# swift-nav/albatross

Hardware: AMD Instinct MI355X
Metric: GP fits/sec (Gram+Chol+solve) at N=16384 fp64 (higher is better)
Workload: dtype f64

## Files before the change

albatross_amd/csrc/api.hip:

```cpp
#include <algorithm>
#include <atomic>
#include <cmath>
#include <cstring>
#include <chrono>
#include <cstdio>
#include <new>
#include <thread>

#include "api_internal.h"
#include "batch_front.h"
#include <deque>
#include <mutex>
#include <tuple>
#include <unordered_map>
#include "trace.h"
#include "pub.h"

namespace agp {

void DeviceFeatures::release() {
  for (void *&p : owned) {
    if (p) (void)hipFree(p);
    p = nullptr;
  }
// ... 138 lines not shown
  return n;
}

static constexpr long long BACKSUB_COOP_MAX_N = 2047;
static agp_context::Tuning read_tuning() {
  agp_context::Tuning t;
  auto flag = [](const char *name, bool dflt) {
    const char *e = getenv(name);
    return e && e[0] ? e[0] == '1' : dflt;
  };
  auto number = [](const char *name, long long dflt) {
    const char *e = getenv(name);
    return e && e[0] ? atoll(e) : dflt;
  };
  t.panel_fused = flag("AGP_PANEL_FUSED", true);
  t.step_below = number("AGP_STEP_BELOW", 4608);
  t.gram_sop = flag("AGP_GRAM_SOP", true);
  t.backsub_coop = flag("AGP_BACKSUB_COOP", true);
  t.backsub_coop_max = number("AGP_BACKSUB_COOP_MAX", BACKSUB_COOP_MAX_N);
  t.mixed_bf16 = flag("AGP_MIXED_BF16", true);
  t.mixed_f16 = flag("AGP_MIXED_F16", true);
  set_f16x2_kernel((int)number("AGP_F16X2_LDS_PAD", 8192), (int)number("AGP_F16X2_TERMS", 4), (int)number("AGP_F16X2_CHUNK", 32));
  t.mixed_nbo = number("AGP_MIXED_NBO", 512);
  t.fp64_nbo = number("AGP_FP64_NBO", 0);
  if (t.fp64_nbo <= 512 || t.fp64_nbo % 128 != 0) t.fp64_nbo = 0;
  set_bf16x3_kernel((int)number("AGP_BF16X3_KERNEL", 2), (int)number("AGP_BF16X3_LDS_PAD", 8192));
  t.sparse_pivoted = flag("AGP_SPARSE_PIVOTED", false);
  t.predict_chunk = number("AGP_PREDICT_CHUNK", 0);
  t.shard_block = number("AGP_SHARD_BLOCK", 0);
  t.shard_force_comm = flag("AGP_SHARD_FORCE_COMM", false);
  t.shard_host_pacing = flag("AGP_SHARD_HOST_PACING", false);
  if (const char *e = getenv("AGP_SHARD_MASK_GFLOP")) t.shard_mask_gflop = atof(e);
  t.merge_above = number("AGP_MERGE_ABOVE", 8704);
  return t;
}

int agp_context_create(int device_id, agp_context **out) {
  if (!out) return AGP_ERR_INVALID_ARGUMENT;
  *out = nullptr;
  int n = 0;
  if (hipGetDeviceCount(&n) != hipSuccess || n <= 0) return AGP_ERR_NO_DEVICE;
  if (device_id < 0 || device_id >= n) return AGP_ERR_INVALID_ARGUMENT;
  agp_context_impl *ctx = new (std::nothrow) agp_context_impl();
  if (!ctx) return AGP_ERR_INVALID_ARGUMENT;
  ctx->device = device_id;
  ctx->tune = read_tuning();
  agp::g_gram_sop = ctx->tune.gram_sop;
  AGP_HIP_CHECK(ctx, hipSetDevice(device_id));
  {
    int lo = 0, hi = 0;
    AGP_HIP_CHECK(ctx, hipDeviceGetStreamPriorityRange(&lo, &hi));
    AGP_HIP_CHECK(ctx, hipStreamCreateWithPriority(&ctx->stream, hipStreamNonBlocking, hi));
    AGP_HIP_CHECK(ctx, hipStreamCreateWithPriority(&ctx->stream2, hipStreamNonBlocking, lo));
    AGP_HIP_CHECK(ctx, hipStreamCreateWithPriority(&ctx->stream3, hipStreamNonBlocking, lo));
    AGP_HIP_CHECK(ctx, hipEventCreateWithFlags(&ctx->ev_inv, hipEventDisableTiming));
    AGP_HIP_CHECK(ctx, hipEventCreateWithFlags(&ctx->ev_c, hipEventDisableTiming));
    int cus = 256;
    (void)hipDeviceGetAttribute(&cus, hipDeviceAttributeMultiprocessorCount, device_id);
    ctx->cus = cus;
    const int keep = cus / 8 * 7 / 8 * 8;
    if (keep > 0 && keep < cus) {
      uint32_t mask[16] = {0};
      for (int i = 0; i < keep && i < 512; ++i) mask[i / 32] |= 1u << (i % 32);
      if (hipExtStreamCreateWithCUMask(&ctx->stream_masked, (uint32_t)((cus + 31) / 32), mask) != hipSuccess) {
        (void)hipGetLastError();
        ctx->stream_masked = nullptr;
// ... 1693 lines not shown
```

albatross_amd/csrc/chol.hip:

```cpp
#include <cstdlib>
#include "common.h"
#include "mfma_f64.h"
#include "gemm_tiles.h"
#include "trsm_kernel.h"
#include "pub.h"
#include "factor_plan.h"

namespace agp {
void launch_set_identity_batched(hipStream_t s, double *B, long long ld, long long stride, long long m, long long count);

__device__ __forceinline__ double readlane_f64(double v, int lane) {
  const long long b = __double_as_longlong(v);
  const int lo = __builtin_amdgcn_readlane((int)(b & 0xffffffffll), lane);
  const int hi = __builtin_amdgcn_readlane((int)(b >> 32), lane);
  return __longlong_as_double(((long long)hi << 32) | (unsigned int)lo);
}

__device__ __forceinline__ double rsqrt_nr(double x) {
  double y = __builtin_amdgcn_rsq(x);
  const double h = 0.5 * x;
  y = y * (1.5 - h * y * y);
  y = y * (1.5 - h * y * y);
  return y;
}
// ... 795 lines not shown
    ctx->d_rowcnt = nullptr;
    ctx->dpub_cap = 0;
    const long long cap = (b1 + 31) / 32 * 32;
    if (hipMalloc(&ctx->d_dpub, sizeof(double) * (size_t)cap * (IMG_DOUBLES + 2)) == hipSuccess) {
      ctx->dpub_cap = cap;
      ctx->d_rowcnt = reinterpret_cast<unsigned long long *>(ctx->d_dpub + cap * (long long)IMG_DOUBLES);
    }
    else (void)hipGetLastError();
  }
  const long long cnt_img = (b1 - b0) * (long long)IMG_DOUBLES, cnt_z = k_end - k_begin;
  if (ctx->d_dpub && ctx->dpub_cap >= b1) {
    prep->fill(ctx->d_rowcnt + 2 * b0, 0ull, 2 * (b1 - b0));
    prep->sentinel(ctx->d_dpub + b0 * (long long)IMG_DOUBLES, cnt_img);
  }
  prep->sentinel(invd + b0 * (long long)IMG_DOUBLES, cnt_img);
  prep->sentinel(ctx->d_zpub + k_begin, cnt_z);
  if (want_step && k_begin == 0 && ctx->d_headcnt && ctx->tune.merge_above > 0 && k_end > ctx->tune.merge_above && !prep->full()) {
    prep->fill(ctx->d_headcnt, 0ull, agp_context::HEADCNT_WORDS);
    ctx->headcnt_ready = true;
  }
  ctx->zpub_ready_n = k_end;
  ctx->img_ready = invd;
  return true;
}

void panel_fused_prepare(agp_context *ctx, hipStream_t s, double *invd, long long k_begin, long long k_end, bool want_step) {
  PrepArgs prep;
  if (panel_fused_plan(ctx, invd, k_begin, k_end, want_step, &prep)) launch_prep(s, prep);
}

static FactorSwitches factor_switches(agp_context *ctx, const double *invd, long long upto, int variant) {
  FactorSwitches sw;
  sw.panel_fused = ctx->tune.panel_fused; sw.step_below = ctx->tune.step_below; sw.merge_above = ctx->tune.merge_above;
  sw.nbo_override = ctx->nbo_override;
  sw.nbo_wide = (variant == 4 || variant == 5) ? ctx->nbo_wide : ctx->tune.fp64_nbo;
  sw.variant = variant;
  sw.step_slots = sw.step_below > 0 ? step_slots(ctx) : 0;
  sw.cus = ctx->cus;
  sw.have_masked_stream = ctx->stream_masked != nullptr;
  sw.headcnt_ready = ctx->headcnt_ready;
  sw.fused_buffers_ready = ctx->d_zpub && ctx->zpub_ready_n >= upto && ctx->img_ready == invd;
  sw.step_buffers_ready = sw.panel_fused && sw.fused_buffers_ready && ctx->d_dpub && ctx->dpub_cap * NB >= upto && ctx->d_rowcnt;
  sw.inv_requested = ctx->bs_W && ctx->ev_inv && ctx->stream2;
  sw.bs_BW = ctx->bs_BW; sw.bs_done = ctx->bs_done;
  return sw;
}

static void panel_phase(agp_context *ctx, hipStream_t s, double *A, long long n, long long lda, double *invd,
                        double *y, long long K0, long long kend, FactorTimers *timers, const FactorSwitches &sw,
                        bool want_step = false, long long mark_after = -1, hipEvent_t mark_event = nullptr) {
  const PanelPlan pp = plan_panels(n, K0, kend, want_step, sw);
  const bool step_mode = pp.step_mode, inner_left = pp.inner_left, fused = pp.fused;
  for (long long k = K0; k < kend; k += NB) {
    const int nbk = (int)((n - k < NB) ? n - k : NB);
    if (mark_event && k == mark_after + NB) (void)hipEventRecord(mark_event, s);
    if (inner_left && k > K0) {
      const double *P = A + K0 * lda + k;
      timed_gemm(s, timers, A + k * lda + k, lda, P, P, n - k, nbk, k - K0, false);
    }
    const long long below = n - (k + nbk);
    if (fused) {
      PotrfArgs pa;
      pa.A = A; pa.lda = lda; pa.k0 = k; pa.nbk = nbk;
      pa.img = invd + (k / NB) * (long long)IMG_DOUBLES;
      pa.y = y ? y + k : nullptr;
      pa.flags = ctx->d_flags; pa.scalars = ctx->d_scalars;
      pa.zpub = y ? ctx->d_zpub + k : nullptr;
      pa.below = below > 0 ? below : 0;
      if (step_mode && k > K0) {
        pa.dpub = ctx->d_dpub + (k / NB) * (long long)IMG_DOUBLES;
        const StepLaunchShape sh = step_launch_shape(pa.below, (k - K0) / NB, sw.step_slots, sw.cus);
        pa.trail_first = sh.trail_first; pa.trail_tiles = sh.trail_tiles; pa.trail_workers = sh.trail_workers;
        pa.hold_index = sh.hold_index; pa.hold_count = sh.hold_count;
        pa.rowcnt_expect = sh.rowcnt_expect;
        if (pa.below > 0) pa.rowcnt = ctx->d_rowcnt + (k + NB) / 64;
        hipLaunchKernelGGL(panel_fused_kernel<true>, dim3(sh.grid), dim3(256), 0, s, pa);
        ++ctx->sched.panels_step;
      } else {
        hipLaunchKernelGGL(panel_fused_kernel<false>, dim3((unsigned)(1 + (pa.below + 63) / 64)), dim3(256), 0, s, pa);
        ++ctx->sched.panels_fused;
      }
      if (below <= 0) continue;
    } else {
      launch_potrf(s, A, lda, k, nbk, invd, y, ctx->d_flags, ctx->d_scalars);
      ++ctx->sched.panels_split;
      if (below <= 0) continue;
      TrsmArgs t;
      t.img = invd + (k / NB) * (long long)IMG_DOUBLES;
      t.nbk = nbk;
      t.Y = A + k * lda + (k + nbk);
      t.stride_m = lda; t.stride_n = 1;
// ... 362 lines not shown
```

albatross_amd/csrc/common.h:

```cpp
#pragma once
#include <hip/hip_runtime.h>
#include <cstdint>
#include <cstdio>
#include <string>
#include <type_traits>
#include <utility>
#include <vector>

#include "../../include/albatross_amd.h"
#include "cov_eval.h"

#define AGP_CHAIN_PRIO 3

namespace agp {

constexpr int NB = 128;
constexpr int NBO = 512;
constexpr int MB = 16;
constexpr int NMB = NB / MB;

template <class F>
inline void dispatch_dim(int dim, F &&f) {
  if (dim == 1) f(std::integral_constant<int, 1>{});
  else if (dim == 2) f(std::integral_constant<int, 2>{});
// ... 55 lines not shown
  size_t pool_aux_bytes = 0;
  int update_variant = -1;
  long long nbo_override = 0;
  long long nbo_wide = 0;
  double *pool_shard = nullptr;
  size_t pool_shard_bytes = 0;
  double *pool_sparse = nullptr;
  size_t pool_sparse_bytes = 0;
  double *pool_batch = nullptr;
  size_t pool_batch_bytes = 0;
  double *d_zpub = nullptr;
  long long zpub_cap = 0, zpub_ready_n = 0;
  double *d_dpub = nullptr;
  long long dpub_cap = 0;
  int cus = 256;
  long long step_slots = 0;
  struct Tuning {
    bool panel_fused = true;
    long long step_below = 4608;
    bool gram_sop = true;
    long long fp64_nbo = 0;
    long long mixed_nbo = 512;
    bool mixed_f16 = true;
    bool mixed_bf16 = true;
    long long backsub_coop_max = 2047;
    bool backsub_coop = true;
    bool sparse_pivoted = false;
    long long predict_chunk = 0;
    long long shard_block = 0;
    bool shard_force_comm = false;
    bool shard_host_pacing = false;
    double shard_mask_gflop = 40.;
    long long merge_above = 8704;
  } tune;
  unsigned long long *d_rowcnt = nullptr;
  void *h_stage = nullptr;
  size_t h_stage_bytes = 0;
  static constexpr long long HEADCNT_WORDS = 256;
  unsigned long long *d_headcnt = nullptr;
  bool headcnt_ready = false;
  struct ScheduleRecord {
    static constexpr unsigned MERGED = 1, STEP = 2, THROTTLED = 4, MASKED = 8, SINGLE = 16;
    enum Backsub { BS_NONE = 0, BS_COOP_DIRECT = 1, BS_COOP_FLAGS = 2, BS_WIDE = 3, BS_CHAIN = 4 };
    static constexpr unsigned INV_EARLY = 1, INV_LAST_STEP = 2, INV_TAIL = 4;
    long long n = 0;
    long long steps = 0, steps_dropped = 0;
    long long kend[HEADCNT_WORDS] = {};
    unsigned bits[HEADCNT_WORDS] = {};
    long long panels_step = 0, panels_fused = 0, panels_split = 0;
    int backsub = BS_NONE;
    long long bs_done = 0;
    unsigned inv_bits = 0;
    int handover_timeout = 0;
    long long demotions = 0;
    void reset_factor(long long n_) {
      n = n_;
      steps = steps_dropped = 0;
      panels_step = panels_fused = panels_split = 0;
      inv_bits = 0;
      handover_timeout = 0;
    }
    void add_step(long long end, unsigned b) {
      if (steps < HEADCNT_WORDS) { kend[steps] = end; bits[steps] = b; ++steps; }
      else ++steps_dropped;
    }
  } sched;
  double *bs_W = nullptr;
  long long bs_BW = 0, bs_done = 0;
  hipEvent_t ev_inv = nullptr;
  const double *img_ready = nullptr;
  bool prep_external = false;
  hipStream_t stream_comm = nullptr;
  unsigned long long *shard_flags = nullptr;
  unsigned long long shard_seq[16] = {};
  unsigned long long shard_probe_seq = 0;
  int shard_host_pacing = -1;
  bool shard_probe_ok = false;
};

struct agp_fit_slab {
  double *base = nullptr;
  size_t bytes = 0;
  int refs = 0;
};

struct agp_fit {
  agp_context *ctx = nullptr;
  agp_fit_slab *slab = nullptr;
  size_t A_bytes = 0;
  int device = 0;
  int64_t n = 0;
// ... 89 lines not shown
void right_solve_lt_batched(hipStream_t s, const double *A, long long stride_A, long long n, long long lda,
                            const double *invd, long long stride_invd, double *X, long long stride_X, long long nrows,
                            long long ldx, long long count);
void launch_gemm_nt_sub_batched(hipStream_t s, double *C, long long ldc, long long batch_C, const double *A,
                                long long lda, bool a_kmajor, long long batch_A, const double *B, long long ldb,
                                bool b_kmajor, long long batch_B, long long M, long long N, long long K, bool tri,
                                long long count);
void right_solve_lt(hipStream_t s, const double *A, long long n, long long lda, const double *invd, double *X,
                    long long nrows, long long ldx);
void forward_solve_mat_lookahead(agp_context *ctx, const double *A, long long n, long long lda, const double *invd,
                                 double *B, long long m, long long ldb, bool rhs_lower = false);
void backward_solve_mat(hipStream_t s, const double *A, long long n, long long lda, const double *invd,
                        double *B, long long m, long long ldb);
constexpr long long WIDE_BW = 512;
bool forward_solve_wide_ok(long long n, long long ncols);
void invert_wide_blocks(hipStream_t s, const double *A, long long n, long long lda, const double *invd, long long BW, double *W);
void forward_solve_wide(hipStream_t s, const double *A, long long n, long long lda, const double *Winv, const double *B,
                        long long ldb, double *X, long long ldx, long long ncols);

void launch_coldot(hipStream_t s, const double *A, long long lda, const double *B, long long ldb,
                   long long n, long long m, double *out, double scale, const double *base);
void launch_gemm_tn_sub(hipStream_t s, const double *V, long long ldv, const double *W, long long ldw,
                        long long n, long long m, double *C, long long ldc);
void launch_gemv_t(hipStream_t s, const double *A, long long lda, long long n, long long m,
                   const double *x, double *y);
void launch_dot(hipStream_t s, const double *a, const double *b, long long n, double *out);

}

namespace agp {
void launch_gemm_nt_sub(hipStream_t s, double *C, long long ldc, const double *A, long long lda,
                        bool a_kmajor, const double *B, long long ldb, bool b_kmajor, long long M,
                        long long N, long long K, bool tri);
void launch_gemm_nt_ext(hipStream_t s, double *C, long long ldc, const double *Cin, long long ldcin, const double *A, long long lda,
                        const double *B, long long ldb, long long M, long long N, long long K);
void launch_gemm_nt_sub_stair(hipStream_t s, double *C, long long ldc, const double *A, long long lda, const double *B,
                              long long ldb, long long M, long long N, long long K, int world, int rank, long long lb0,
                              long long block, long long c0);
struct BulkTiming {
  hipEvent_t e0 = nullptr, e1 = nullptr;
  double flops = 0.;
};
void launch_trailing_update_as(int variant, hipStream_t s, double *C, long long ldc, const double *P,
                               const double *Q, long long ldp, long long M, long long K,
                               BulkTiming *timing = nullptr, const float *P32 = nullptr, const float *Q32 = nullptr,
                               long long ld32 = 0);
void launch_trailing_update(hipStream_t s, double *C, long long ldc, const double *P, const double *Q,
                            long long ldp, long long M, long long K, BulkTiming *timing = nullptr);
void read_bulk_probe(unsigned long long *out);
void read_bf16_probe(unsigned long long *out);
void read_potrf_probe(unsigned long long *out);
void launch_head_gate(hipStream_t s, const unsigned long long *done, unsigned long long expect, int *flags);
void launch_trailing_update_merged(hipStream_t s, double *C, long long ldc, const double *P, long long ldp, long long M, long long K,
                                   int head_cols, unsigned long long *head_done, long long *head_tiles, BulkTiming *timing = nullptr);
void launch_update_f32(hipStream_t s, double *C, long long ldc, const double *P, const double *Q, long long ldp, long long M,
                       long long N, long long K, const float *P32 = nullptr, const float *Q32 = nullptr, long long ld32 = 0);
size_t bf16x3_bytes(long long rows, long long K);
void launch_convert_panel_bf16x3(hipStream_t s, const double *P, long long ldp, long long rows, long long K, unsigned short *planes);
void set_bf16x3_kernel(int choice, int lds_pad);
void launch_update_bf16x3(hipStream_t s, double *C, long long ldc, const unsigned short *planes, long long panel_rows, long long row_a,
                          long long row_b, long long M, long long N, long long K, const int *order = nullptr, long long order_len = 0);
size_t f16x2_bytes(long long rows, long long K);
void launch_f16x2_row_scales(hipStream_t s, const double *A, long long lda, long long n, double *rs, double *irs);
void launch_convert_panel_f16x2(hipStream_t s, const double *P, long long ldp, long long rows, long long K, const double *rs,
                                unsigned short *planes);
void set_f16x2_kernel(int lds_pad, int terms, int chunk);
// ... 8 lines not shown
```

albatross_amd/csrc/debug_api.hip:

```cpp
#include <algorithm>
#include <cstdio>
#include "common.h"
#include "api_internal.h"
#include "mfma_f64.h"
#include "shard_internal.h"
#include "pub.h"
#include "trsm_kernel.h"
#include "factor_plan.h"
#include <cstdlib>
#include <cstring>
#include <new>

#define AGP_DEBUG_API __attribute__((visibility("default")))

namespace agp {

__global__ void mfma_tile_kernel(const double *A, const double *B, double *D) {
  const int l = threadIdx.x;
  v4d acc = v4zero();
  acc = mfma16(A[(l & 15) * 4 + (l >> 4)], B[(l >> 4) * 16 + (l & 15)], acc);
  for (int r = 0; r < 4; ++r) D[((l >> 4) + 4 * r) * 16 + (l & 15)] = acc[r];
}

template <int NACC>
// ... 519 lines not shown
  AGP_HIP_CHECK(ctx, hipEventElapsedTime(&ms, e0, e1));
  std::vector<unsigned long long> h(2 * nblk);
  AGP_HIP_CHECK(ctx, hipMemcpy(h.data(), d, sizeof(unsigned long long) * 2 * nblk, hipMemcpyDeviceToHost));
  std::vector<double> cyc(nblk), clk(nblk);
  for (int i = 0; i < nblk; ++i) {
    cyc[i] = (double)h[2 * i] / (double)iters;
    clk[i] = (double)h[2 * i] / ((double)h[2 * i + 1] * 10.0);
  }
  std::sort(cyc.begin(), cyc.end());
  std::sort(clk.begin(), clk.end());
  out[0] = cyc[nblk / 2];
  out[1] = clk[nblk / 2];
  out[2] = (double)nblk * 4.0 * iters * (nm * 2048.0 + nv * 128.0) / (ms * 1e-3) / 1e12;
  out[3] = nm; out[4] = nv;
  (void)hipEventDestroy(e0); (void)hipEventDestroy(e1); (void)hipFree(d);
  return AGP_OK;
}

AGP_DEBUG_API int agp_debug_gemm(agp_context *ctx, double *C, int64_t ldc, const double *A, int64_t lda, int a_kmajor,
                   const double *B, int64_t ldb, int b_kmajor, int64_t M, int64_t N, int64_t K, int tri) {
  if (!ctx) return AGP_ERR_INVALID_ARGUMENT;
  AGP_HIP_CHECK(ctx, hipSetDevice(ctx->device));
  const size_t cb = sizeof(double) * (size_t)ldc * (size_t)N;
  const size_t ab = sizeof(double) * (size_t)lda * (size_t)(a_kmajor ? M : K);
  const size_t bb = sizeof(double) * (size_t)ldb * (size_t)(b_kmajor ? N : K);
  double *dC = nullptr, *dA = nullptr, *dB = nullptr;
  AGP_HIP_CHECK(ctx, hipMalloc(&dC, cb));
  AGP_HIP_CHECK(ctx, hipMalloc(&dA, ab));
  AGP_HIP_CHECK(ctx, hipMalloc(&dB, bb));
  AGP_HIP_CHECK(ctx, hipMemcpy(dC, C, cb, hipMemcpyHostToDevice));
  AGP_HIP_CHECK(ctx, hipMemcpy(dA, A, ab, hipMemcpyHostToDevice));
  AGP_HIP_CHECK(ctx, hipMemcpy(dB, B, bb, hipMemcpyHostToDevice));
  launch_gemm_nt_sub(ctx->stream, dC, ldc, dA, lda, a_kmajor != 0, dB, ldb, b_kmajor != 0, M, N, K, tri != 0);
  AGP_HIP_CHECK(ctx, hipStreamSynchronize(ctx->stream));
  AGP_HIP_CHECK(ctx, hipGetLastError());
  AGP_HIP_CHECK(ctx, hipMemcpy(C, dC, cb, hipMemcpyDeviceToHost));
  (void)hipFree(dC); (void)hipFree(dA); (void)hipFree(dB);
  return AGP_OK;
}

AGP_DEBUG_API int agp_debug_fmac_rate(agp_context *ctx, int waves_per_simd, int mode, int iters, double *out, double *probe) {
  if (!ctx) return AGP_ERR_INVALID_ARGUMENT;
  AGP_HIP_CHECK(ctx, hipSetDevice(ctx->device));
  const int nblk = 256 * waves_per_simd;
  unsigned long long *d = nullptr;
  double *dp = nullptr;
  AGP_HIP_CHECK(ctx, hipMalloc(&d, sizeof(unsigned long long) * 2 * nblk));
  AGP_HIP_CHECK(ctx, hipMalloc(&dp, sizeof(double) * 64));
  hipEvent_t e0, e1;
  AGP_HIP_CHECK(ctx, hipEventCreate(&e0));
  AGP_HIP_CHECK(ctx, hipEventCreate(&e1));
  for (int rep = 0; rep < 2; ++rep) {
    AGP_HIP_CHECK(ctx, hipEventRecord(e0, ctx->stream));
    if (mode == 0) hipLaunchKernelGGL(fmac_rate_kernel<0>, dim3(nblk), dim3(256), 0, ctx->stream, d, dp, iters, 1.1);
    else if (mode == 1) hipLaunchKernelGGL(fmac_rate_kernel<1>, dim3(nblk), dim3(256), 0, ctx->stream, d, dp, iters, 1.1);
    else hipLaunchKernelGGL(fmac_rate_kernel<2>, dim3(nblk), dim3(256), 0, ctx->stream, d, dp, iters, 1.1);
    AGP_HIP_CHECK(ctx, hipEventRecord(e1, ctx->stream));
    AGP_HIP_CHECK(ctx, hipEventSynchronize(e1));
  }
  float ms = 0.f;
  AGP_HIP_CHECK(ctx, hipEventElapsedTime(&ms, e0, e1));
  std::vector<unsigned long long> h(2 * nblk);
  AGP_HIP_CHECK(ctx, hipMemcpy(h.data(), d, sizeof(unsigned long long) * 2 * nblk, hipMemcpyDeviceToHost));
  if (probe) AGP_HIP_CHECK(ctx, hipMemcpy(probe, dp, sizeof(double) * 64, hipMemcpyDeviceToHost));
  std::vector<double> cyc(nblk), clk(nblk);
  for (int i = 0; i < nblk; ++i) {
// ... 472 lines not shown
    AGP_HIP_CHECK(ctx, hipMemcpy(dy, y, sizeof(double) * (size_t)n, hipMemcpyHostToDevice));
  }
  AGP_HIP_CHECK(ctx, hipMemsetAsync(ctx->d_flags, 0, 4 * sizeof(int), ctx->stream));
  AGP_HIP_CHECK(ctx, hipMemsetAsync(ctx->d_scalars, 0, 4 * sizeof(double), ctx->stream));
  factor_lower(ctx, dA, n, lda, dI, dy, nullptr);
  AGP_HIP_CHECK(ctx, hipStreamSynchronize(ctx->stream));
  AGP_HIP_CHECK(ctx, hipGetLastError());
  AGP_HIP_CHECK(ctx, hipMemcpy(A, dA, ab, hipMemcpyDeviceToHost));
  if (y) AGP_HIP_CHECK(ctx, hipMemcpy(y, dy, sizeof(double) * (size_t)n, hipMemcpyDeviceToHost));
  int flags[4];
  double scal[4];
  AGP_HIP_CHECK(ctx, hipMemcpy(flags, ctx->d_flags, sizeof(flags), hipMemcpyDeviceToHost));
  AGP_HIP_CHECK(ctx, hipMemcpy(scal, ctx->d_scalars, sizeof(scal), hipMemcpyDeviceToHost));
  if (log_det) *log_det = 2. * scal[0];
  if (bad_pivot) *bad_pivot = flags[1] ? flags[1] - 1 : -1;
  (void)hipFree(dA); (void)hipFree(dI);
  if (dy) (void)hipFree(dy);
  ctx->sched.backsub = agp_context::ScheduleRecord::BS_NONE;
  ctx->sched.bs_done = 0;
  ctx->sched.handover_timeout = flags[2];
  return AGP_OK;
}

constexpr int64_t SCHED_HEADER = 20;
AGP_DEBUG_API int agp_debug_schedule(agp_context *ctx, int64_t *out, int64_t cap) {
  if (!ctx || !out || cap < 0) return AGP_ERR_INVALID_ARGUMENT;
  const agp_context::ScheduleRecord &r = ctx->sched;
  int64_t w[SCHED_HEADER + 2 * agp_context::HEADCNT_WORDS] = {};
  w[0] = r.n; w[1] = r.steps; w[2] = r.steps_dropped;
  w[3] = r.panels_step; w[4] = r.panels_fused; w[5] = r.panels_split;
  w[6] = r.backsub; w[7] = r.bs_done; w[8] = r.inv_bits; w[9] = r.handover_timeout; w[10] = r.demotions;
  w[11] = ctx->step_slots; w[12] = ctx->cus; w[13] = ctx->stream_masked ? 1 : 0;
  w[14] = ctx->tune.step_below; w[15] = ctx->tune.panel_fused ? 1 : 0; w[16] = ctx->tune.merge_above;
  w[17] = ctx->tune.backsub_coop ? 1 : 0; w[18] = ctx->tune.fp64_nbo;
  for (long long i = 0; i < r.steps; ++i) {
    w[SCHED_HEADER + 2 * i] = r.kend[i];
    w[SCHED_HEADER + 2 * i + 1] = r.bits[i];
  }
  const int64_t total = SCHED_HEADER + 2 * agp_context::HEADCNT_WORDS;
  for (int64_t i = 0; i < cap && i < total; ++i) out[i] = w[i];
  return AGP_OK;
}

constexpr int64_t PLAN_WORDS = SCHED_HEADER + 7 * agp_context::HEADCNT_WORDS;
AGP_DEBUG_API int agp_debug_factor_plan(const int64_t *switches, int64_t n, int64_t *out, int64_t cap) {
  if (!switches || !out || n < 1 || cap < 0) return AGP_ERR_INVALID_ARGUMENT;
  agp::FactorSwitches sw;
  sw.panel_fused = switches[0] != 0; sw.step_below = switches[1]; sw.merge_above = switches[2];
  sw.nbo_override = switches[3]; sw.nbo_wide = switches[4]; sw.variant = (int)switches[5];
  sw.step_slots = switches[6]; sw.cus = switches[7];
  sw.have_masked_stream = switches[8] != 0; sw.headcnt_ready = switches[9] != 0;
  sw.step_buffers_ready = switches[10] != 0; sw.fused_buffers_ready = switches[11] != 0;
  sw.inv_requested = switches[12] != 0; sw.bs_BW = switches[13]; sw.bs_done = switches[14];
  int64_t w[PLAN_WORDS] = {};
  int64_t *steps = w + SCHED_HEADER, *intents = steps + 2 * agp_context::HEADCNT_WORDS;
  agp::FactorPlanner plan(n, sw);
  agp::OuterStep s;
  w[0] = n;
  while (plan.next(s)) {
    const int64_t blocks = (s.next_end - s.kend + agp::NB - 1) / agp::NB;
    const agp::PanelPlan pp = agp::plan_panels(n, s.kend, s.next_end, s.step_mode, sw);
    if (!pp.fused) w[5] += blocks;
    else if (!pp.step_mode) w[4] += blocks;
    else { w[4] += 1; w[3] += blocks - 1; }
    w[8] |= (s.inv_last_step > 0 ? agp::INV_BIT_LAST_STEP : 0u) | (s.inv_count > 0 ? s.inv_bit : 0u);
    plan.inversion_under_panels(s, s.inv_count > 0);
    if (w[1] >= agp_context::HEADCNT_WORDS) { ++w[2]; continue; }
    const int64_t i = w[1]++;
    steps[2 * i] = s.next_end; steps[2 * i + 1] = s.bits;
    const int64_t intent[5] = {s.inv_last_step, s.inv_first, s.inv_count, s.mark_after, s.inv_bit};
    std::copy(intent, intent + 5, intents + 5 * i);
  }
  w[7] = plan.bs_done();
  std::copy(w, w + std::min(cap, PLAN_WORDS), out);
  return AGP_OK;
}

AGP_DEBUG_API int agp_debug_step_launch_shape(int64_t below, int64_t panels_done, int64_t step_slots, int64_t cus, int64_t *out) {
  if (!out || below < 0) return AGP_ERR_INVALID_ARGUMENT;
  const agp::StepLaunchShape sh = agp::step_launch_shape(below, panels_done, step_slots, cus);
  const int64_t w[7] = {sh.grid, sh.trail_first, sh.trail_tiles, sh.trail_workers, sh.hold_index, sh.hold_count, (int64_t)sh.rowcnt_expect};
  std::copy(w, w + 7, out);
  return AGP_OK;
}

}

namespace agp {
__global__ __launch_bounds__(256) void mfma_peak_kernel(double *sink, int iters, double a0, double b0) {
  v4d acc[8];
#pragma unroll
  for (int i = 0; i < 8; ++i) acc[i] = v4zero();
  double a = a0 + threadIdx.x * 1e-9, b = b0 - threadIdx.x * 1e-9;
  for (int it = 0; it < iters; ++it) {
#pragma unroll
    for (int i = 0; i < 8; ++i) acc[i] = mfma16(a, b, acc[i]);
  }
  double s = 0.;
#pragma unroll
  for (int i = 0; i < 8; ++i) s += acc[i][0] + acc[i][1] + acc[i][2] + acc[i][3];
  if (s == 123.456) sink[0] = s;
}

static int mfma_f64_peak(hipStream_t s, int iters, double *tflops) {
  double *sink = nullptr;
  if (hipMalloc(&sink, 8) != hipSuccess) return AGP_ERR_HIP;
  hipEvent_t e0, e1;
  (void)hipEventCreate(&e0);
  (void)hipEventCreate(&e1);
  const int blocks = 256 * 2;
// ... 182 lines not shown
```

albatross_amd/csrc/factor_plan.h:

```cpp
#pragma once

namespace agp {

constexpr long long FUSED_BELOW = 4608;
constexpr long long INNER_LEFT_ABOVE = 6144;
constexpr long long NBO_512_ABOVE = 2048, NBO_256_ABOVE = 1024;
constexpr long long NBO_WIDE_ABOVE = 8192;
constexpr long long THROTTLE_BELOW = 8192;
constexpr long long U1_F32_ABOVE = 4096;
constexpr long long SINGLE_BELOW = 1536;
constexpr long long MASK_BELOW = 8704;
constexpr long long HANDOVER_BULK_ABOVE = 1536;
constexpr long long PLAN_NB = 128;
constexpr long long STEP_FIXED_CRITICAL = 10;
constexpr long long MERGED_STEPS_MAX = 256;

struct FactorSwitches {
  bool panel_fused = true;
  long long step_below = 4608, merge_above = 8704;
  long long nbo_override = 0, nbo_wide = 0;
  int variant = -1;
  long long step_slots = 0, cus = 256;
  bool have_masked_stream = false;
  bool headcnt_ready = false;
  bool step_buffers_ready = false;
  bool fused_buffers_ready = false;
  bool inv_requested = false;
  long long bs_BW = 0, bs_done = 0;
};

constexpr unsigned STEP_BIT_MERGED = 1, STEP_BIT_STEP = 2, STEP_BIT_THROTTLED = 4, STEP_BIT_MASKED = 8, STEP_BIT_SINGLE = 16;
constexpr unsigned INV_BIT_EARLY = 1, INV_BIT_LAST_STEP = 2, INV_BIT_TAIL = 4;

struct OuterStep {
  long long k0 = 0, kend = 0, next_end = 0;
  long long index = 0;
  unsigned bits = 0;
  bool step_mode = false;
  bool masked = false;
  bool mixed_tall = false;
  bool handover_whole_trailing = false;
  long long inv_last_step = 0;
  long long inv_first = 0, inv_count = 0, mark_after = -1;
  unsigned inv_bit = 0;
};

inline bool step_fits(long long step_below, long long step_slots, long long rows) {
  return step_below > 0 && rows <= step_below && step_slots >= STEP_FIXED_CRITICAL + rows / 64 + 64;
}

inline long long pick_nbo(long long remaining, long long override_nbo, long long wide) {
  if (override_nbo > 0) return override_nbo;
// ... 40 lines not shown
      s.handover_whole_trailing = step && rows > HANDOVER_BULK_ABOVE;
      s.bits = (step ? STEP_BIT_STEP : 0u) | (throttle ? STEP_BIT_THROTTLED : 0u) | (single ? STEP_BIT_SINGLE : 0u) |
               (!last && s.masked ? STEP_BIT_MASKED : 0u);
      if (step && bs_done_ > 0 && last_wide > bs_done_ && bs_done_ == kend_ / bw && last_wide * bw - PLAN_NB >= kend_)
        under_panels(s, bs_done_, last_wide - bs_done_, INV_BIT_TAIL);
    }
    k0_ = kend_;
    kend_ = s.next_end;
    return true;
  }

  void inversion_under_panels(const OuterStep &s, bool ran) { if (ran) bs_done_ = s.inv_first + s.inv_count; }
  long long bs_done() const { return bs_done_; }

 private:
  bool invertible() const { return sw_.inv_requested && sw_.bs_BW > 0; }
  bool step_ok(long long rows) const {
    return sw_.nbo_override == 0 && step_fits(sw_.step_below, sw_.step_slots, rows) && sw_.step_buffers_ready;
  }
  long long clip(long long end) const { return end > n_ ? n_ : end; }
  void under_panels(OuterStep &s, long long first, long long count, unsigned bit) const {
    s.inv_first = first; s.inv_count = count; s.inv_bit = bit;
    s.mark_after = (first + count) * sw_.bs_BW - PLAN_NB;
  }
  const long long n_;
  const FactorSwitches sw_;
  long long k0_ = 0, kend_ = 0, index_ = 0, bs_done_;
  bool started_ = false;
};

struct PanelPlan {
  bool step_mode;
  bool inner_left;
  bool fused;
};

inline PanelPlan plan_panels(long long n, long long k0, long long kend, bool step_mode, const FactorSwitches &sw) {
  PanelPlan p;
  p.step_mode = step_mode && kend == n;
  p.inner_left = !p.step_mode && (n - k0) > INNER_LEFT_ABOVE;
  p.fused = sw.panel_fused && sw.fused_buffers_ready && ((n - k0) <= FUSED_BELOW || p.step_mode);
  return p;
}

struct StepLaunchShape {
  unsigned grid = 0, trail_first = 0xffffffffu, hold_index = 0xffffffffu, hold_count = 0;
  long long trail_tiles = 0, trail_workers = 1;
  unsigned long long rowcnt_expect = 0;
};

inline StepLaunchShape step_launch_shape(long long below, long long panels_done, long long step_slots, long long cus) {
  StepLaunchShape sh;
  sh.grid = (unsigned)(STEP_FIXED_CRITICAL + (below + 63) / 64);
  if (below <= 0) return sh;
  const long long nt = (below + 63) / 64;
  sh.trail_first = sh.grid;
  sh.rowcnt_expect = 2ull * (unsigned long long)panels_done;
  const long long tiles = nt * (nt + 1) / 2 + 2 * nt;
  const long long slots = step_slots, first_round = cus, ncrit = sh.grid;
  long long workers = tiles, nhold = 0;
  if (ncrit + workers > first_round && ncrit < first_round) {
    nhold = tiles <= 1200 ? ncrit : STEP_FIXED_CRITICAL;
    const long long cap = slots - ncrit - nhold;
    if (workers > cap) workers = cap;
    if (ncrit + workers <= first_round) nhold = 0;
  } else if (workers > slots - ncrit) {
    workers = slots - ncrit;
  }
  if (workers < 2 * nt) workers = 2 * nt < tiles ? 2 * nt : tiles;
  sh.trail_tiles = tiles;
  sh.trail_workers = workers;
  sh.grid += (unsigned)workers;
  if (nhold > 0) {
    sh.hold_index = (unsigned)first_round;
    sh.hold_count = (unsigned)nhold;
// ... 7 lines not shown
```

albatross_amd/csrc/gemm.hip:

```cpp
#include <cmath>
#include <cstdlib>
#include <algorithm>
#include <map>
#include <mutex>
#include <tuple>
#include <vector>
#include "common.h"
#include "mfma_f64.h"
#include "gemm_tiles.h"

namespace agp {




__device__ __forceinline__ bool tile_of_block(const GemmArgs &g, int &bi, int &bj) {
  if (g.stair) {
    const long long id = blockIdx.x;
    bi = (int)(id % g.ntr);
    bj = (int)(id / g.ntr);
    const long long lb = g.st_lb0 + bi / g.st_tpb;
    const long long gi = lb * g.st_world + ((lb & 1) ? g.st_world - 1 - g.st_rank : g.st_rank);
    return bj <= gi * g.st_tpb - g.st_c0t + (bi % g.st_tpb);
  }
// ... 415 lines not shown
  if (b_kmajor && !tri && tiles * count < small_limit) {
    GemmArgs h = g;
    h.a_kmajor = a_kmajor ? 1 : 0;
    h.ntr = (int)((M + ST - 1) / ST);
    h.ntc = (int)((N + ST - 1) / ST);
    hipLaunchKernelGGL(gemm64_nt_sub_bk_kernel, dim3((unsigned)((long long)h.ntr * h.ntc), (unsigned)count), dim3(GEMM_THREADS), 0, s,
                       h);
    return;
  }
  if (!a_kmajor && !b_kmajor && tiles * count < small_limit) {
    GemmArgs h = g;
    h.ntr = (int)((M + ST - 1) / ST);
    h.ntc = (int)((N + ST - 1) / ST);
    if (tri && h.ntc > h.ntr) h.ntc = h.ntr;
    const long long t64 = count_tiles(h.ntr, h.ntc, h.tri);
    if (t64 * count < 256 && K >= 256) {
      h.ntr = (int)((M + TT - 1) / TT);
      h.ntc = (int)((N + TT - 1) / TT);
      if (tri && h.ntc > h.ntr) h.ntc = h.ntr;
      const long long t32 = count_tiles(h.ntr, h.ntc, h.tri);
      hipLaunchKernelGGL(gemm32_nt_sub_kernel, dim3((unsigned)t32, (unsigned)count), dim3(GEMM_THREADS), 0, s, h);
      return;
    }
    hipLaunchKernelGGL(gemm64_nt_sub_kernel, dim3((unsigned)t64, (unsigned)count), dim3(GEMM_THREADS), 0, s, h);
    return;
  }
  dim3 grid((unsigned)tiles, (unsigned)count), block(GEMM_THREADS);
  if (!a_kmajor && !b_kmajor) hipLaunchKernelGGL((gemm_nt_sub_kernel<false, false>), grid, block, 0, s, g);
  else if (!a_kmajor && b_kmajor) hipLaunchKernelGGL((gemm_nt_sub_kernel<false, true>), grid, block, 0, s, g);
  else if (a_kmajor && !b_kmajor) hipLaunchKernelGGL((gemm_nt_sub_kernel<true, false>), grid, block, 0, s, g);
  else hipLaunchKernelGGL((gemm_nt_sub_kernel<true, true>), grid, block, 0, s, g);
}

void launch_gemm_nt_sub_stair(hipStream_t s, double *C, long long ldc, const double *A, long long lda, const double *B,
                              long long ldb, long long M, long long N, long long K, int world, int rank, long long lb0,
                              long long block, long long c0) {
  if (M <= 0 || N <= 0 || K <= 0) return;
  GemmArgs g;
  g.C = C; g.ldc = ldc; g.A = A; g.lda = lda; g.B = B; g.ldb = ldb;
  g.M = M; g.N = N; g.K = K; g.tri = 0;
  g.ntr = (int)((M + GT - 1) / GT);
  g.ntc = (int)((N + GT - 1) / GT);
  g.stair = 1; g.st_world = world; g.st_rank = rank; g.st_tpb = (int)(block / GT);
  g.st_lb0 = lb0; g.st_c0t = c0 / GT;
  static int slots = 0;
  if (slots == 0) {
    int dev = 0, cus = 256;
    if (hipGetDevice(&dev) != hipSuccess || hipDeviceGetAttribute(&cus, hipDeviceAttributeMultiprocessorCount, dev) != hipSuccess || cus <= 0)
      cus = 256;
    slots = 2 * cus;
  }
  if ((long long)g.ntr * g.ntc / 2 < 4LL * slots) {
    g.ntr = (int)((M + ST - 1) / ST);
    g.ntc = (int)((N + ST - 1) / ST);
    g.st_tpb = (int)(block / ST);
    g.st_c0t = c0 / ST;
    hipLaunchKernelGGL(gemm64_nt_sub_kernel, dim3((unsigned)((long long)g.ntr * g.ntc)), dim3(GEMM_THREADS), 0, s, g);
    return;
  }
  hipLaunchKernelGGL((gemm_nt_sub_kernel<false, false>), dim3((unsigned)((long long)g.ntr * g.ntc)), dim3(GEMM_THREADS), 0, s, g);
}

void launch_gemm_nt_ext(hipStream_t s, double *C, long long ldc, const double *Cin, long long ldcin, const double *A, long long lda,
                        const double *B, long long ldb, long long M, long long N, long long K) {
  if (M <= 0 || N <= 0 || K <= 0) return;
  GemmArgs g;
// ... 215 lines not shown
```

Baseline: 34.77.

## Aggregate inner left-looking panel updates into 256-wide mid-level GEMMs

In the left-looking inner panel loop, the trailing update is split into two levels. Every 256 columns one wider GEMM applies all earlier panels to the next 256-column strip, using a 128-tile kernel. Panels in between only receive a short update from the panels since the last 256 boundary. This replaces many thin, deep GEMMs with fewer wider ones to improve reuse and occupancy, at the cost of a new launch path and more tuning knobs.

```diff
diff --git a/albatross_amd/csrc/api.hip b/albatross_amd/csrc/api.hip
--- a/albatross_amd/csrc/api.hip
+++ b/albatross_amd/csrc/api.hip
@@ -194,6 +194,9 @@
   t.shard_host_pacing = flag("AGP_SHARD_HOST_PACING", false);
   if (const char *e = getenv("AGP_SHARD_MASK_GFLOP")) t.shard_mask_gflop = atof(e);
   t.merge_above = number("AGP_MERGE_ABOVE", 8704);
+  t.inner_mid = flag("AGP_INNER_MID", t.inner_mid);
+  t.inner_left_above = number("AGP_INNER_LEFT_ABOVE", t.inner_left_above);
+  if (t.inner_left_above < 0) t.inner_left_above = 0;
   return t;
 }
 
diff --git a/albatross_amd/csrc/chol.hip b/albatross_amd/csrc/chol.hip
--- a/albatross_amd/csrc/chol.hip
+++ b/albatross_amd/csrc/chol.hip
@@ -851,6 +851,7 @@
 static FactorSwitches factor_switches(agp_context *ctx, const double *invd, long long upto, int variant) {
   FactorSwitches sw;
   sw.panel_fused = ctx->tune.panel_fused; sw.step_below = ctx->tune.step_below; sw.merge_above = ctx->tune.merge_above;
+  sw.inner_mid = ctx->tune.inner_mid; sw.inner_left_above = ctx->tune.inner_left_above;
   sw.nbo_override = ctx->nbo_override;
   sw.nbo_wide = (variant == 4 || variant == 5) ? ctx->nbo_wide : ctx->tune.fp64_nbo;
   sw.variant = variant;
@@ -873,9 +874,15 @@
   for (long long k = K0; k < kend; k += NB) {
     const int nbk = (int)((n - k < NB) ? n - k : NB);
     if (mark_event && k == mark_after + NB) (void)hipEventRecord(mark_event, s);
-    if (inner_left && k > K0) {
-      const double *P = A + K0 * lda + k;
-      timed_gemm(s, timers, A + k * lda + k, lda, P, P, n - k, nbk, k - K0, false);
+    const PanelProduct q = panel_product(n, K0, kend, k, pp);
+    if (q.kind != PRODUCT_NONE) {
+      const double *P = A + (k - q.depth) * lda + k;
+      if (q.kind == PRODUCT_MID) {
+        launch_gemm_nt_sub_tile128(s, A + k * lda + k, lda, P, lda, P, lda, n - k, q.width, q.depth, true);
+        ++ctx->sched.mid_updates;
+      } else {
+        timed_gemm(s, timers, A + k * lda + k, lda, P, P, n - k, q.width, q.depth, false);
+      }
     }
     const long long below = n - (k + nbk);
     if (fused) {
diff --git a/albatross_amd/csrc/common.h b/albatross_amd/csrc/common.h
--- a/albatross_amd/csrc/common.h
+++ b/albatross_amd/csrc/common.h
@@ -111,6 +111,8 @@
     bool shard_host_pacing = false;
     double shard_mask_gflop = 40.;
     long long merge_above = 8704;
+    bool inner_mid = true;
+    long long inner_left_above = 6144;
   } tune;
   unsigned long long *d_rowcnt = nullptr;
   void *h_stage = nullptr;
@@ -127,6 +129,7 @@
     long long kend[HEADCNT_WORDS] = {};
     unsigned bits[HEADCNT_WORDS] = {};
     long long panels_step = 0, panels_fused = 0, panels_split = 0;
+    long long mid_updates = 0;
     int backsub = BS_NONE;
     long long bs_done = 0;
     unsigned inv_bits = 0;
@@ -135,7 +138,7 @@
     void reset_factor(long long n_) {
       n = n_;
       steps = steps_dropped = 0;
-      panels_step = panels_fused = panels_split = 0;
+      panels_step = panels_fused = panels_split = mid_updates = 0;
       inv_bits = 0;
       handover_timeout = 0;
     }
@@ -291,6 +294,8 @@
 void launch_gemm_nt_sub(hipStream_t s, double *C, long long ldc, const double *A, long long lda,
                         bool a_kmajor, const double *B, long long ldb, bool b_kmajor, long long M,
                         long long N, long long K, bool tri);
+void launch_gemm_nt_sub_tile128(hipStream_t s, double *C, long long ldc, const double *A, long long lda, const double *B,
+                                long long ldb, long long M, long long N, long long K, bool tri);
 void launch_gemm_nt_ext(hipStream_t s, double *C, long long ldc, const double *Cin, long long ldcin, const double *A, long long lda,
                         const double *B, long long ldb, long long M, long long N, long long K);
 void launch_gemm_nt_sub_stair(hipStream_t s, double *C, long long ldc, const double *A, long long lda, const double *B,
diff --git a/albatross_amd/csrc/debug_api.hip b/albatross_amd/csrc/debug_api.hip
--- a/albatross_amd/csrc/debug_api.hip
+++ b/albatross_amd/csrc/debug_api.hip
@@ -575,6 +575,28 @@
   AGP_HIP_CHECK(ctx, hipMemcpy(dA, A, ab, hipMemcpyHostToDevice));
   AGP_HIP_CHECK(ctx, hipMemcpy(dB, B, bb, hipMemcpyHostToDevice));
   launch_gemm_nt_sub(ctx->stream, dC, ldc, dA, lda, a_kmajor != 0, dB, ldb, b_kmajor != 0, M, N, K, tri != 0);
+  AGP_HIP_CHECK(ctx, hipStreamSynchronize(ctx->stream));
+  AGP_HIP_CHECK(ctx, hipGetLastError());
+  AGP_HIP_CHECK(ctx, hipMemcpy(C, dC, cb, hipMemcpyDeviceToHost));
+  (void)hipFree(dC); (void)hipFree(dA); (void)hipFree(dB);
+  return AGP_OK;
+}
+
+AGP_DEBUG_API int agp_debug_gemm_tile128(agp_context *ctx, double *C, int64_t ldc, const double *A, int64_t lda, const double *B,
+                                         int64_t ldb, int64_t M, int64_t N, int64_t K, int tri) {
+  if (!ctx || !C || !A || !B || M < 1 || N < 1 || K < 1 || ldc < M || lda < M || ldb < N) return AGP_ERR_INVALID_ARGUMENT;
+  AGP_HIP_CHECK(ctx, hipSetDevice(ctx->device));
+  const size_t cb = sizeof(double) * (size_t)ldc * (size_t)N;
+  const size_t ab = sizeof(double) * (size_t)lda * (size_t)K;
+  const size_t bb = sizeof(double) * (size_t)ldb * (size_t)K;
+  double *dC = nullptr, *dA = nullptr, *dB = nullptr;
+  AGP_HIP_CHECK(ctx, hipMalloc(&dC, cb));
+  AGP_HIP_CHECK(ctx, hipMalloc(&dA, ab));
+  AGP_HIP_CHECK(ctx, hipMalloc(&dB, bb));
+  AGP_HIP_CHECK(ctx, hipMemcpy(dC, C, cb, hipMemcpyHostToDevice));
+  AGP_HIP_CHECK(ctx, hipMemcpy(dA, A, ab, hipMemcpyHostToDevice));
+  AGP_HIP_CHECK(ctx, hipMemcpy(dB, B, bb, hipMemcpyHostToDevice));
+  launch_gemm_nt_sub_tile128(ctx->stream, dC, ldc, dA, lda, dB, ldb, M, N, K, tri != 0);
   AGP_HIP_CHECK(ctx, hipStreamSynchronize(ctx->stream));
   AGP_HIP_CHECK(ctx, hipGetLastError());
   AGP_HIP_CHECK(ctx, hipMemcpy(C, dC, cb, hipMemcpyDeviceToHost));
@@ -1113,7 +1135,7 @@
   w[6] = r.backsub; w[7] = r.bs_done; w[8] = r.inv_bits; w[9] = r.handover_timeout; w[10] = r.demotions;
   w[11] = ctx->step_slots; w[12] = ctx->cus; w[13] = ctx->stream_masked ? 1 : 0;
   w[14] = ctx->tune.step_below; w[15] = ctx->tune.panel_fused ? 1 : 0; w[16] = ctx->tune.merge_above;
-  w[17] = ctx->tune.backsub_coop ? 1 : 0; w[18] = ctx->tune.fp64_nbo;
+  w[17] = ctx->tune.backsub_coop ? 1 : 0; w[18] = ctx->tune.fp64_nbo; w[19] = r.mid_updates;
   for (long long i = 0; i < r.steps; ++i) {
     w[SCHED_HEADER + 2 * i] = r.kend[i];
     w[SCHED_HEADER + 2 * i + 1] = r.bits[i];
@@ -1157,6 +1179,24 @@
   return AGP_OK;
 }
 
+AGP_DEBUG_API int64_t agp_debug_panel_products(int64_t n, int64_t k0, int64_t kend, int inner_left, int inner_mid, int64_t *out, int64_t cap) {
+  if (n < 1 || k0 < 0 || kend <= k0 || kend > n || k0 % agp::PLAN_NB != 0 || (!out && cap > 0)) return -1;
+  agp::PanelPlan pp;
+  pp.step_mode = false; pp.fused = false;
+  pp.inner_left = inner_left != 0; pp.inner_mid = pp.inner_left && inner_mid != 0;
+  int64_t count = 0;
+  for (long long k = k0; k < kend; k += agp::PLAN_NB) {
+    const agp::PanelProduct q = agp::panel_product(n, k0, kend, k, pp);
+    if (q.kind == agp::PRODUCT_NONE) continue;
+    if (count < cap) {
+      const int64_t w[4] = {k, q.kind, q.depth, q.width};
+      std::copy(w, w + 4, out + 4 * count);
+    }
+    ++count;
+  }
+  return count;
+}
+
 AGP_DEBUG_API int agp_debug_step_launch_shape(int64_t below, int64_t panels_done, int64_t step_slots, int64_t cus, int64_t *out) {
   if (!out || below < 0) return AGP_ERR_INVALID_ARGUMENT;
   const agp::StepLaunchShape sh = agp::step_launch_shape(below, panels_done, step_slots, cus);
diff --git a/albatross_amd/csrc/factor_plan.h b/albatross_amd/csrc/factor_plan.h
--- a/albatross_amd/csrc/factor_plan.h
+++ b/albatross_amd/csrc/factor_plan.h
@@ -4,6 +4,7 @@
 
 constexpr long long FUSED_BELOW = 4608;
 constexpr long long INNER_LEFT_ABOVE = 6144;
+constexpr long long INNER_SUB = 256;
 constexpr long long NBO_512_ABOVE = 2048, NBO_256_ABOVE = 1024;
 constexpr long long NBO_WIDE_ABOVE = 8192;
 constexpr long long THROTTLE_BELOW = 8192;
@@ -18,6 +19,8 @@
 struct FactorSwitches {
   bool panel_fused = true;
   long long step_below = 4608, merge_above = 8704;
+  bool inner_mid = true;
+  long long inner_left_above = INNER_LEFT_ABOVE;
   long long nbo_override = 0, nbo_wide = 0;
   int variant = -1;
   long long step_slots = 0, cus = 256;
@@ -124,15 +127,37 @@
 struct PanelPlan {
   bool step_mode;
   bool inner_left;
+  bool inner_mid;
   bool fused;
 };
 
 inline PanelPlan plan_panels(long long n, long long k0, long long kend, bool step_mode, const FactorSwitches &sw) {
   PanelPlan p;
   p.step_mode = step_mode && kend == n;
-  p.inner_left = !p.step_mode && (n - k0) > INNER_LEFT_ABOVE;
+  p.inner_left = !p.step_mode && (n - k0) > sw.inner_left_above;
+  p.inner_mid = p.inner_left && sw.inner_mid;
   p.fused = sw.panel_fused && sw.fused_buffers_ready && ((n - k0) <= FUSED_BELOW || p.step_mode);
   return p;
+}
+
+constexpr int PRODUCT_NONE = 0, PRODUCT_NEAR = 1, PRODUCT_MID = 2;
+struct PanelProduct {
+  int kind = PRODUCT_NONE;
+  long long depth = 0, width = 0;
+};
+
+inline PanelProduct panel_product(long long n, long long k0, long long kend, long long k, const PanelPlan &pp) {
+  PanelProduct q;
+  const long long off = k - k0, nbk = n - k < PLAN_NB ? n - k : PLAN_NB;
+  if (!pp.inner_left || off <= 0 || k >= kend) return q;
+  if (!pp.inner_mid) {
+    q.kind = PRODUCT_NEAR; q.depth = off; q.width = nbk;
+  } else if (off % INNER_SUB == 0) {
+    q.kind = PRODUCT_MID; q.depth = off; q.width = kend - k < INNER_SUB ? kend - k : INNER_SUB;
+  } else {
+    q.kind = PRODUCT_NEAR; q.depth = off % INNER_SUB; q.width = nbk;
+  }
+  return q;
 }
 
 struct StepLaunchShape {
diff --git a/albatross_amd/csrc/gemm.hip b/albatross_amd/csrc/gemm.hip
--- a/albatross_amd/csrc/gemm.hip
+++ b/albatross_amd/csrc/gemm.hip
@@ -471,6 +471,20 @@
   else hipLaunchKernelGGL((gemm_nt_sub_kernel<true, true>), grid, block, 0, s, g);
 }
 
+void launch_gemm_nt_sub_tile128(hipStream_t s, double *C, long long ldc, const double *A, long long lda, const double *B,
+                                long long ldb, long long M, long long N, long long K, bool tri) {
+  if (M <= 0 || N <= 0 || K <= 0) return;
+  GemmArgs g;
+  g.C = C; g.ldc = ldc; g.A = A; g.lda = lda; g.B = B; g.ldb = ldb;
+  g.M = M; g.N = N; g.K = K; g.tri = tri ? 1 : 0;
+  g.ntr = (int)((M + GT - 1) / GT);
+  g.ntc = (int)((N + GT - 1) / GT);
+  if (tri && g.ntc > g.ntr) g.ntc = g.ntr;
+  const long long tiles = count_tiles(g.ntr, g.ntc, g.tri);
+  if (tiles <= 0) return;
+  hipLaunchKernelGGL((gemm_nt_sub_kernel<false, false>), dim3((unsigned)tiles), dim3(GEMM_THREADS), 0, s, g);
+}
+
 void launch_gemm_nt_sub_stair(hipStream_t s, double *C, long long ldc, const double *A, long long lda, const double *B,
                               long long ldb, long long M, long long N, long long K, int world, int rank, long long lb0,
                               long long block, long long c0) {
```

Result: no change. 34.98 (median of 6 runs) (+0.6%).
